# bluenote-1577/sylph

Measured on NVIDIA H100. Metric: bases/s sketched, higher is better.
Workload: dtype u64

## Files before the change

### sylph_b200/csrc/common.cuh

```cuda
#pragma once

#include <cuda_runtime.h>

#include <algorithm>
#include <stdint.h>
#include <stdio.h>

#include <string>
#include <unordered_map>
#include <utility>
#include <vector>

#include "../../include/sylph_b200.h"

namespace syl {

void set_error(const std::string &msg);

struct Status {
    int code;
    Status(int c = SYL_OK) : code(c) {}
    bool ok() const { return code == SYL_OK; }
};

#define SYL_CUDA(call)                                                                           \
    do {                                                                                         \
        cudaError_t _e = (call);                                                                 \
        if (_e != cudaSuccess) {                                                                 \
            ::syl::set_error(std::string(#call) + ": " + cudaGetErrorString(_e) + " (" +       \
                             __FILE__ + ":" + std::to_string(__LINE__) + ")");                   \
            return (_e == cudaErrorMemoryAllocation) ? SYL_ERR_OOM : SYL_ERR_CUDA;               \
        }                                                                                        \
    } while (0)

#define SYL_TRY(expr)                                                                            \
    do {                                                                                         \
        int _s = (expr);                                                                         \
        if (_s != SYL_OK) return _s;                                                             \
    } while (0)

}

struct syl_ctx {
    int device = 0;
    cudaStream_t stream = nullptr;
    bool own_stream = false;
    int num_sms = 132;
    uint64_t launches = 0;
    uint64_t *d_counters = nullptr;
    uint64_t *h_counters = nullptr;
    bool timing = false;
    struct TimedLaunch { int which; cudaEvent_t e0, e1; };
    std::vector<TimedLaunch> timed_pending;
    std::vector<cudaEvent_t> event_pool;
    double kernel_ms[SYL_KERNEL_COUNT] = {};
    uint64_t kernel_launches[SYL_KERNEL_COUNT] = {};
    uint64_t seed_bases = 0;
    uint64_t ingest_h2d_bytes = 0, ingest_chunks_packed = 0, ingest_chunks_ascii = 0;
    void *ingest = nullptr;
    cudaStream_t copy_stream = nullptr;
    cudaEvent_t ev_copied[2] = {nullptr, nullptr}, ev_used[2] = {nullptr, nullptr};
    uint8_t *stage_b[2] = {nullptr, nullptr};
    uint64_t *stage_o[2] = {nullptr, nullptr};
    uint64_t stage_cap_b[2] = {0, 0}, stage_cap_o[2] = {0, 0};
    std::vector<std::pair<void *, size_t>> free_blocks;
    std::unordered_map<void *, size_t> handle_blocks;
    size_t cached_bytes = 0;
};

namespace syl {
struct KernelTimer {
    syl_ctx *c;
    int which;
    cudaEvent_t e0 = nullptr, e1 = nullptr;
    KernelTimer(syl_ctx *ctx, int w) : c(ctx), which(w) {
        if (!c->timing) return;
        auto take = [&]() {
            cudaEvent_t e = nullptr;
            if (!c->event_pool.empty()) { e = c->event_pool.back(); c->event_pool.pop_back(); }
            else if (cudaEventCreate(&e) != cudaSuccess) e = nullptr;
            return e;
        };
        e0 = take(); e1 = take();
        if (e0 && e1) cudaEventRecord(e0, c->stream);
    }
    void stop() {
        if (!e0 || !e1) return;
        cudaEventRecord(e1, c->stream);
        c->timed_pending.push_back({which, e0, e1});
        e0 = e1 = nullptr;
    }
    ~KernelTimer() { stop(); }
};
extern thread_local syl_ctx *tl_ctx;
int hblock_alloc(syl_ctx *ctx, void **p, size_t bytes);
void hblock_free(syl_ctx *ctx, void *p);
}

struct syl_sample {
    int device = 0;
    syl_ctx *owner = nullptr;
    cudaStream_t stream = nullptr;
    uint64_t *hash = nullptr;
    uint32_t *count = nullptr;
    uint64_t n = 0;
    int k = 31;
    uint64_t c = 200;
    double mean_read_length = 0.;
    uint64_t num_dup_removed = 0;
    uint64_t sum_counts = 0;
    bool sum_counts_valid = false;
};

struct syl_genomes {
    int device = 0;
    syl_ctx *owner = nullptr;
    cudaStream_t stream = nullptr;
    uint64_t n = 0;
    uint64_t *kmers = nullptr, *kmer_off = nullptr;
    uint64_t *tracked = nullptr, *tracked_off = nullptr;
    uint64_t *gn_size = nullptr;
    uint64_t total_kmers = 0, total_tracked = 0;
    int has_tracked = 0;
    int k = 31;
    uint64_t c = 200;
};

namespace syl {

struct EventRec { uint64_t hash, recflag, p0, p1; };
static_assert(sizeof(EventRec) == 32, "EventRec is one 32-byte sector");
constexpr uint64_t NO_PAIR = 1ull;
constexpr uint64_t EV_PENDING = 1ull << 63;

constexpr uint32_t GRP_BPG = 32;

struct SeedJob {
    const uint8_t *d_bases = nullptr;
    const uint32_t *d_packed = nullptr;
    uint64_t n_bases = 0;
    const uint64_t *d_rec_off = nullptr;
    uint64_t off_bias = 0, n_rec = 0;
    int k = 31;
    uint64_t c = 200;
    int sem = SYL_SEM_AVX2, with_pos = 0;
    void *d_out = nullptr;
    uint64_t cap = 0;
    int emit_events = 0;
    uint64_t rec_base = 0;
    int no_dedup = 0;
    uint32_t *d_pend = nullptr;
    uint32_t *d_group_cnt = nullptr;
    uint64_t Mb = 0;
    uint32_t nbk = 0, ng = 0, slot = 0;
    unsigned long long *d_count = nullptr, *d_pend_count = nullptr;
    uint32_t slot_cap = 0;
    uint32_t *d_tile_cnt = nullptr, *d_slot_overflow = nullptr;
};
uint64_t seed_cta_tiles(uint64_t n_bases);
uint64_t seed_cta_tile_bases();
bool seed_cta_kernel_selected();
int seed_enqueue(syl_ctx *ctx, const SeedJob &job);
void ingest_destroy(syl_ctx *ctx);

template <typename T>
struct DevBuf {
    T *p = nullptr;
    size_t n = 0, cap_bytes = 0;
    cudaStream_t s = nullptr;
    syl_ctx *owner = nullptr;
    DevBuf() {}
    DevBuf(const DevBuf &) = delete;
    DevBuf &operator=(const DevBuf &) = delete;
    ~DevBuf() { release(); }
    int alloc(size_t count, cudaStream_t stream) {
        release();
        s = stream;
        n = count;
        size_t bytes = (std::max<size_t>(count, 1) * sizeof(T) + 255) & ~(size_t)255;
        syl_ctx *c = tl_ctx;
        owner = c;
        if (c) {
            size_t best = (size_t)-1, bi = 0;
            for (size_t i = 0; i < c->free_blocks.size(); i++) {
                const size_t sz = c->free_blocks[i].second;
                if (sz >= bytes && sz < best) { best = sz; bi = i; }
            }
            if (best != (size_t)-1 && best <= 2 * bytes + (1u << 20)) {
                p = reinterpret_cast<T *>(c->free_blocks[bi].first);
                cap_bytes = best;
                c->free_blocks[bi] = c->free_blocks.back();
                c->free_blocks.pop_back();
                return SYL_OK;
            }
        }
        cudaError_t e = cudaMalloc((void **)&p, bytes);
        if (e != cudaSuccess) {
            p = nullptr;
            set_error(std::string("cudaMalloc(") + std::to_string(bytes) + " B): " + cudaGetErrorString(e));
            return e == cudaErrorMemoryAllocation ? SYL_ERR_OOM : SYL_ERR_CUDA;
        }
        cap_bytes = bytes;
        if (c) c->cached_bytes += bytes;
        return SYL_OK;
    }
    void swap(DevBuf &o) {
        std::swap(p, o.p); std::swap(n, o.n); std::swap(cap_bytes, o.cap_bytes); std::swap(s, o.s); std::swap(owner, o.owner);
    }
    void release() {
        if (p) {
            if (owner) owner->free_blocks.emplace_back((void *)p, cap_bytes);
            else cudaFree(p);
        }
        p = nullptr;
        n = 0;
    }
};

__device__ __forceinline__ uint32_t even_fields(uint64_t x) {
    x &= 0xCCCCCCCCCCCCCCCCull;
    x = (x | (x << 2)) & 0xF0F0F0F0F0F0F0F0ull;
    x = (x | (x << 4)) & 0xFF00FF00FF00FF00ull;
    x = (x | (x << 8)) & 0xFFFF0000FFFF0000ull;
    x = (x | (x << 16)) & 0xFFFFFFFF00000000ull;
    return (uint32_t)(x >> 32);
}


__host__ __device__ __forceinline__ uint32_t byte_to_seq(uint32_t b) {
    switch (b) {
        case 1: case 'C': case 'c': return 1u;
        case 2: case 'G': case 'g': return 2u;
        case 3: case 'T': case 't': case 'U': case 'u': return 3u;
        default: return 0u;
    }
}

__host__ __device__ __forceinline__ uint64_t mm_hash64(uint64_t key) {
    key = ~(key * 0x200001ull);
    key ^= key >> 24;
    key *= 265ull;
    key ^= key >> 14;
    key *= 21ull;
    key ^= key >> 28;
    key *= 0x80000001ull;
    return key;
}

__host__ __device__ __forceinline__ uint64_t fmh_threshold(uint64_t c) {
    return 0xFFFFFFFFFFFFFFFFull / c;
}

__host__ __device__ __forceinline__ uint64_t valid_windows(uint64_t L, uint32_t k, int sem,
                                                           int with_pos) {
    if (L < k) return 0;
    if (sem == SYL_SEM_SCALAR) return L - k + 1;
    uint64_t min_len = with_pos ? 2ull * k : (uint64_t)k + 1;
    if (L < min_len) return 0;
    return 4ull * ((L - k + 1) / 4);
}

}
```

### sylph_b200/csrc/seed_kernel.cuh

```cuda
#pragma once
#include "common.cuh"

namespace syl {

constexpr int SEED_THREADS = 256;
#ifndef SEED_TILE_CFG
#define SEED_TILE_CFG 32768
#endif
#ifndef SEED_CANON_MODE
#define SEED_CANON_MODE 3
#endif
#ifndef SEED_MINB_CFG
#define SEED_MINB_CFG 4
#endif
constexpr int SEED_TILE = SEED_TILE_CFG;
constexpr int SEED_W_MAX = 32;
constexpr int SEED_W_MIN = 24;
constexpr int SEED_HALO = 48;
constexpr int SEED_STAGE = SEED_TILE >= 32768 ? 512 : 256;
constexpr int SEED_CAND = SEED_TILE >= 32768 ? 1024 : 512;
constexpr int SEED_RUNS_PER_THREAD = (SEED_TILE / SEED_W_MIN + 2 * SEED_THREADS - 1) / SEED_THREADS;
constexpr int SEED_MAXRUNS = SEED_THREADS * SEED_RUNS_PER_THREAD;
static_assert(SEED_MAXRUNS >= SEED_TILE / SEED_W_MIN + SEED_THREADS, "run table too small");
constexpr int SEED_ASC_BYTES = SEED_TILE + SEED_HALO;
constexpr int SEED_NCHUNK16 = SEED_ASC_BYTES / 16;
constexpr int SEED_FW_WORDS = SEED_NCHUNK16 + 1 + 8;
constexpr int SEED_CW_WORDS = SEED_NCHUNK16 + 8;

struct SeedSmem {
    alignas(128) uint8_t asc[SEED_ASC_BYTES + 16];
    alignas(16) uint32_t fw[SEED_FW_WORDS];
    alignas(16) uint32_t cw[SEED_CW_WORDS];
    alignas(16) uint8_t lut[4][256];
    alignas(8) unsigned long long mbar;
};
struct SeedMeta {
    long long rel[SEED_THREADS];
    int s0[SEED_THREADS];
    int cnt[SEED_THREADS];
    int len[SEED_THREADS];
    int rbase[SEED_THREADS + 1];
    int warp_tot[SEED_THREADS / 32];
    unsigned int stage_count;
    unsigned int cand_count;
    unsigned long long flush_base;
    alignas(16) EventRec stage[SEED_STAGE];
    uint32_t cand[SEED_CAND];
    uint16_t run_rec[SEED_MAXRUNS];
};
static_assert(sizeof(SeedMeta) <= SEED_ASC_BYTES, "meta must fit in the dead ASCII region");
static_assert(SEED_TILE <= 65536, "tile-relative window starts are kept as u16");
__device__ __forceinline__ uint16_t *seed_stage_pos(SeedMeta &M) {
    return reinterpret_cast<uint16_t *>(reinterpret_cast<syl_survivor *>(M.stage) + SEED_STAGE);
}

struct GroupOut {
    uint32_t *cnt;
    uint64_t Mb;
    uint32_t nbk, ng, slot;
    __device__ __forceinline__ uint64_t place(uint64_t h, unsigned long long *g_count, uint64_t cap) const {
        if (cnt) {
            uint32_t g = (uint32_t)__umul64hi(h, Mb);
            g = (g < nbk ? g : nbk - 1) / GRP_BPG;
            const uint32_t i = atomicAdd(&cnt[g], 1u);
            if (i < slot) return (uint64_t)g * slot + i;
        }
        const unsigned long long gi = atomicAdd(g_count, 1ull);
        return gi < cap ? (uint64_t)ng * slot + gi : ~0ull;
    }
};

struct ShiftMul { uint32_t m24, m14, m28, one, zero; };

struct SlotOut { uint32_t cap; uint32_t *tile_cnt; uint32_t *overflow; };

__device__ __forceinline__ void mul64c(uint32_t lo, uint32_t hi, uint32_t c, uint32_t &plo, uint32_t &phi) {
    uint64_t t;
    asm("mul.wide.u32 %0, %1, %2;" : "=l"(t) : "r"(lo), "r"(c));
    plo = (uint32_t)t;
    asm("mad.lo.u32 %0, %1, %2, %3;" : "=r"(phi) : "r"(hi), "r"(c), "r"((uint32_t)(t >> 32)));
}

template <int VAR, int SH>
__device__ __forceinline__ void xorshift(uint32_t &lo, uint32_t &hi, uint32_t mul, uint32_t extra_hi) {
    uint32_t sl, sh;
    if (VAR >= 1) sh = __umulhi(hi, mul); else sh = hi >> SH;
    if (VAR >= 2) sl = __umulhi(lo, mul) + hi * mul; else sl = __funnelshift_r(lo, hi, SH);
    lo ^= sl;
    hi = hi ^ sh ^ extra_hi;
}

template <int VAR>
__device__ __forceinline__ uint32_t hash_hi32(uint32_t lo, uint32_t hi, const ShiftMul sm) {
    uint32_t a, b;
    mul64c(lo, hi, 0x200001u, a, b);
    xorshift<VAR, 24>(a, b, sm.m24, 0xFFFFFF00u);
    mul64c(a, b, 265u, lo, hi);
    xorshift<VAR, 14>(lo, hi, sm.m14, 0u);
    mul64c(lo, hi, 21u, a, b);
    xorshift<VAR, 28>(a, b, sm.m28, 0u);
    return __umulhi(a, 0x80000001u) + b * 0x80000001u;
}

__device__ __forceinline__ uint32_t smem_u32(const void *p) {
    return (uint32_t)__cvta_generic_to_shared(p);
}

__device__ __forceinline__ uint64_t fw64(const SeedSmem &S, uint32_t q) {
    const uint32_t bitpos = 32u + 2u * q, w = bitpos >> 5, sh = bitpos & 31u;
    const uint32_t a = S.fw[w], b = S.fw[w + 1], c = S.fw[w + 2];
    return ((uint64_t)__funnelshift_l(b, a, sh) << 32) | __funnelshift_l(c, b, sh);
}

template <int K, int EMIT>
__device__ __forceinline__ void seed_resolve(const SeedSmem &S, SeedMeta &M, uint32_t pw, int j, uint64_t rc, uint64_t thr,
                                             void *__restrict__ out, uint64_t cap,
                                             unsigned long long *__restrict__ g_count, uint64_t rec_base, int no_dedup,
                                             uint32_t *__restrict__ pend, const GroupOut go) {
    constexpr uint32_t PAD = 64 - 2 * K;
    constexpr uint32_t HI_MASK = (1u << (32 - PAD)) - 1u;
    const uint32_t bitpos = 32u + 2u * pw - PAD;
    const uint32_t q0 = bitpos >> 5, sh = bitpos & 31u;
    const uint32_t w0 = S.fw[q0], w1 = S.fw[q0 + 1], w2 = S.fw[q0 + 2];
    const uint64_t f = ((uint64_t)(__funnelshift_l(w1, w0, sh) & HI_MASK) << 32) | __funnelshift_l(w2, w1, sh);
    const uint32_t cq = pw >> 4, csh = (pw & 15u) * 2u;
    const uint32_t c0 = S.cw[cq], c1 = S.cw[cq + 1], c2 = S.cw[cq + 2];
    const uint64_t rr = ((uint64_t)(__funnelshift_r(c1, c2, csh) & HI_MASK) << 32) | __funnelshift_r(c0, c1, csh);
    const uint64_t h = mm_hash64(f < rr ? f : rr);
    if (h >= thr) return;
    const unsigned int idx = atomicAdd(&M.stage_count, 1u);
    if (EMIT == 0) {
        syl_survivor sv;
        sv.hash = h;
        sv.rec = (uint32_t)(rc + (uint64_t)j);
        sv.pos = (uint32_t)((long long)pw - M.rel[j] + (K - 1));
        if (idx < (unsigned)SEED_STAGE) {
            reinterpret_cast<syl_survivor *>(M.stage)[idx] = sv;
            seed_stage_pos(M)[idx] = (uint16_t)pw;
        } else {
            const unsigned long long gi = atomicAdd(g_count, 1ull);
            if (gi < cap) reinterpret_cast<syl_survivor *>(out)[gi] = sv;
        }
    } else {
        EventRec ev;
        ev.hash = h;
        const int L = M.len[j];
        const bool has_pair = !no_dedup && L <= 400 && L >= 66;
        ev.recflag = ((rec_base + rc + (uint64_t)j) << 1) | (no_dedup == 2 ? EV_PENDING : (has_pair ? 0ull : NO_PAIR));
        ev.p0 = 0;
        ev.p1 = 0;
        if (has_pair) {
            const long long st = M.rel[j];
            const long long mid = st + (L >> 1);
            if (st >= 0 && mid + 32 <= (long long)SEED_NCHUNK16 * 16) {
                const uint64_t a = fw64(S, (uint32_t)st), b = fw64(S, (uint32_t)mid);
                const uint32_t kf = even_fields(a), kg = even_fields(a << 2);
                const uint32_t kr = even_fields(b), kt = even_fields(b << 2);
                ev.p0 = ((uint64_t)kf << 32) | kr;
                ev.p1 = ((uint64_t)kg << 32) | kt;
            } else {
                ev.recflag |= EV_PENDING;
            }
        }
        if (idx < (unsigned)SEED_STAGE) {
            M.stage[idx] = ev;
        } else {
            const uint64_t pos = go.place(ev.hash, g_count, cap);
            if (pos != ~0ull) {
                reinterpret_cast<EventRec *>(out)[pos] = ev;
                if (ev.recflag & EV_PENDING) pend[atomicAdd(g_count + 1, 1ull)] = (uint32_t)pos;
            }
        }
    }
}

template <int K, int VAR, int EMIT, int W>
__global__ void __launch_bounds__(SEED_THREADS, SEED_MINB_CFG)
k_seed(const uint8_t *__restrict__ bases, uint64_t n_bases, const uint64_t *__restrict__ rec_off, uint64_t off_bias,
       const uint32_t *__restrict__ tile_rec, uint64_t thr, int sem, int with_pos,
       void *__restrict__ out, uint64_t cap, unsigned long long *__restrict__ g_count,
       const ShiftMul smul, uint64_t rec_base, int no_dedup, uint32_t *__restrict__ pend, const GroupOut go, const SlotOut slot) {
    static_assert(W >= SEED_W_MIN && W <= SEED_W_MAX, "run length");
    extern __shared__ __align__(128) uint8_t smem_raw[];
    SeedSmem &S = *reinterpret_cast<SeedSmem *>(smem_raw);
    SeedMeta &M = *reinterpret_cast<SeedMeta *>(S.asc);

    constexpr uint32_t PAD = 64 - 2 * K;
    constexpr uint32_t HI_MASK = (1u << (32 - PAD)) - 1u;
    const int tid = threadIdx.x;
    const uint64_t T0 = (uint64_t)blockIdx.x * SEED_TILE;
    const uint64_t T1 = T0 + SEED_TILE;
    const uint32_t thr_hi = (uint32_t)(thr >> 32);

    const uint64_t remain = n_bases - T0;
    const uint32_t avail = remain < (uint64_t)SEED_ASC_BYTES ? (uint32_t)remain : (uint32_t)SEED_ASC_BYTES;
    const uint32_t nbulk = avail & ~15u;
    const uint32_t mbar = smem_u32(&S.mbar);
    if (tid == 0) {
        asm volatile("mbarrier.init.shared::cta.b64 [%0], 1;" ::"r"(mbar));
        asm volatile("fence.mbarrier_init.release.cluster;" ::: "memory");
    }
    __syncthreads();
    if (tid == 0 && nbulk) {
        asm volatile("mbarrier.arrive.expect_tx.shared::cta.b64 _, [%0], %1;" ::"r"(mbar), "r"(nbulk)
                     : "memory");
        asm volatile(
            "cp.async.bulk.shared::cluster.global.mbarrier::complete_tx::bytes [%0], [%1], %2, [%3];" ::"r"(
                smem_u32(S.asc)),
            "l"(bases + T0), "r"(nbulk), "r"(mbar)
            : "memory");
    }
    for (uint32_t i = nbulk + tid; i < (uint32_t)SEED_ASC_BYTES + 16; i += SEED_THREADS)
        S.asc[i] = (i < avail) ? bases[T0 + i] : (uint8_t)0;
    {
        const uint32_t code = byte_to_seq((uint32_t)tid);
        S.lut[0][tid] = (uint8_t)(code << 6);
        S.lut[1][tid] = (uint8_t)(code << 4);
        S.lut[2][tid] = (uint8_t)(code << 2);
        S.lut[3][tid] = (uint8_t)code;
    }
    if (tid < 8) {
        S.fw[SEED_NCHUNK16 + 1 + tid] = 0u;
        S.cw[SEED_NCHUNK16 + tid] = 0u;
    }
    if (tid == 0) S.fw[0] = 0u;
    if (nbulk) {
        uint32_t done = 0;
        while (!done) {
            asm volatile(
                "{\n\t.reg .pred p;\n\t"
                "mbarrier.try_wait.parity.shared::cta.b64 p, [%1], 0;\n\t"
                "selp.u32 %0, 1, 0, p;\n\t}"
                : "=r"(done)
                : "r"(mbar)
                : "memory");
        }
    }
    __syncthreads();

    for (int ch = tid; ch < SEED_NCHUNK16; ch += SEED_THREADS) {
        const uint4 v = *reinterpret_cast<const uint4 *>(S.asc + 16 * ch);
        const uint32_t w[4] = {v.x, v.y, v.z, v.w};
        uint32_t g[4];
#pragma unroll
        for (int q = 0; q < 4; q++) {
            const uint32_t b0 = __byte_perm(w[q], 0u, 0x4440), b1 = __byte_perm(w[q], 0u, 0x4441);
            const uint32_t b2 = __byte_perm(w[q], 0u, 0x4442), b3 = __byte_perm(w[q], 0u, 0x4443);
            g[q] = ((uint32_t)S.lut[0][b0] | (uint32_t)S.lut[1][b1] | (uint32_t)S.lut[2][b2]) | (uint32_t)S.lut[3][b3];
        }
        const uint32_t lo16 = __byte_perm(g[3], g[2], 0x0040), hi16 = __byte_perm(g[1], g[0], 0x0040);
        const uint32_t f = __byte_perm(lo16, hi16, 0x5410);
        uint32_t x = __brev(f);
        x = ((x >> 1) & 0x55555555u) | ((x & 0x55555555u) << 1);
        S.fw[1 + ch] = f;
        S.cw[ch] = ~x;
    }
    __syncthreads();

    if (tid == 0) M.stage_count = 0u;

    const uint32_t r_lo = tile_rec[blockIdx.x];
    const uint32_t r_hi = tile_rec[blockIdx.x + 1];
    const int lane = tid & 31, wid = tid >> 5;

    for (uint64_t rc = r_lo; rc <= (uint64_t)r_hi; rc += SEED_THREADS) {
        int runs = 0;
        const uint64_t r = rc + tid;
        if (r <= (uint64_t)r_hi) {
            const uint64_t a = rec_off[r] - off_bias, b = rec_off[r + 1] - off_bias;
            const uint64_t L = b - a;
            const uint64_t nv = valid_windows(L, (uint32_t)K, sem, with_pos);
            const uint64_t lo = a > T0 ? a : T0;
            uint64_t hi = a + nv;
            if (hi > T1) hi = T1;
            const int cnt = hi > lo ? (int)(hi - lo) : 0;
            M.rel[tid] = (long long)a - (long long)T0;
            M.s0[tid] = (int)(lo - T0);
            M.cnt[tid] = cnt;
            M.len[tid] = L > 0x7FFFFFFFull ? 0x7FFFFFFF : (int)L;
            runs = (cnt + W - 1) / W;
        }
        int incl = runs;
#pragma unroll
        for (int d = 1; d < 32; d <<= 1) {
            int t = __shfl_up_sync(0xffffffffu, incl, d);
            if (lane >= d) incl += t;
        }
        if (lane == 31) M.warp_tot[wid] = incl;
        __syncthreads();
        int wbase = 0;
#pragma unroll
        for (int w = 0; w < SEED_THREADS / 32; w++) wbase += (w < wid) ? M.warp_tot[w] : 0;
        M.rbase[tid] = wbase + incl - runs;
        if (tid == SEED_THREADS - 1) M.rbase[SEED_THREADS] = wbase + incl;
        __syncthreads();
        const int total = M.rbase[SEED_THREADS];

        {
            const int base5 = tid * SEED_RUNS_PER_THREAD;
#pragma unroll
            for (int e = 0; e < SEED_RUNS_PER_THREAD; e++) M.run_rec[base5 + e] = 0;
            __syncthreads();
            if (runs > 0) M.run_rec[M.rbase[tid]] = (uint16_t)(tid + 1);
            __syncthreads();
            int v[SEED_RUNS_PER_THREAD], m = 0;
#pragma unroll
            for (int e = 0; e < SEED_RUNS_PER_THREAD; e++) { m = max(m, (int)M.run_rec[base5 + e]); v[e] = m; }
            int inc = m;
#pragma unroll
            for (int d = 1; d < 32; d <<= 1) inc = max(inc, __shfl_up_sync(0xffffffffu, inc, d));
            int excl = __shfl_up_sync(0xffffffffu, inc, 1);
            if (lane == 0) excl = 0;
            if (lane == 31) M.warp_tot[wid] = inc;
            __syncthreads();
            int wmax = 0;
#pragma unroll
            for (int w = 0; w < SEED_THREADS / 32; w++) wmax = max(wmax, (w < wid) ? M.warp_tot[w] : 0);
            const int pre = max(excl, wmax);
#pragma unroll
            for (int e = 0; e < SEED_RUNS_PER_THREAD; e++) M.run_rec[base5 + e] = (uint16_t)max(v[e], pre);
            if (tid == 0) M.cand_count = 0u;
            __syncthreads();
        }

        for (int q = tid; q < total; q += SEED_THREADS) {
            const int j = (int)M.run_rec[q] - 1;
            const int ridx = q - M.rbase[j];
            const int p = M.s0[j] + ridx * W;
            const int n = min(W, M.cnt[j] - ridx * W);

            uint32_t F[4], G[4];
            {
                const uint32_t bitpos = 32u + 2u * (uint32_t)p - PAD;
                const uint32_t q0 = bitpos >> 5, sh = bitpos & 31u;
                uint32_t w0 = S.fw[q0], w1 = S.fw[q0 + 1], w2 = S.fw[q0 + 2], w3 = S.fw[q0 + 3],
                         w4 = S.fw[q0 + 4];
                F[0] = __funnelshift_l(w1, w0, sh);
                F[1] = __funnelshift_l(w2, w1, sh);
                F[2] = __funnelshift_l(w3, w2, sh);
                F[3] = __funnelshift_l(w4, w3, sh);
                const uint32_t cq = (uint32_t)p >> 4, csh = ((uint32_t)p & 15u) * 2u;
                uint32_t c0 = S.cw[cq], c1 = S.cw[cq + 1], c2 = S.cw[cq + 2], c3 = S.cw[cq + 3],
                         c4 = S.cw[cq + 4];
                G[0] = __funnelshift_r(c0, c1, csh);
                G[1] = __funnelshift_r(c1, c2, csh);
                G[2] = __funnelshift_r(c2, c3, csh);
                G[3] = __funnelshift_r(c3, c4, csh);
            }
            uint32_t cand = 0u;
#pragma unroll
            for (int i = 0; i < W; i++) {
                const int jb = (2 * i) >> 5;
                const uint32_t sft = (uint32_t)((2 * i) & 31);
                const uint32_t f_hi = __funnelshift_l(F[jb + 1], F[jb], sft) & HI_MASK;
                const uint32_t f_lo = __funnelshift_l(F[jb + 2], F[jb + 1], sft);
                const uint32_t r_lo = __funnelshift_r(G[jb], G[jb + 1], sft);
                const uint32_t r_hi = __funnelshift_r(G[jb + 1], G[jb + 2], sft) & HI_MASK;
                uint32_t c_lo, c_hi;
#if SEED_CANON_MODE == 0
                const uint64_t f = ((uint64_t)f_hi << 32) | f_lo, rr = ((uint64_t)r_hi << 32) | r_lo;
                const uint64_t canon = f < rr ? f : rr;
                c_lo = (uint32_t)canon; c_hi = (uint32_t)(canon >> 32);
#elif SEED_CANON_MODE == 1
                asm("{\n\t.reg .pred p;\n\t.reg .f64 a, b;\n\tmov.b64 a, {%2, %3};\n\tmov.b64 b, {%4, %5};\n\t"
                    "setp.lt.f64 p, a, b;\n\tselp.b32 %0, %2, %4, p;\n\tselp.b32 %1, %3, %5, p;\n\t}"
                    : "=r"(c_lo), "=r"(c_hi) : "r"(f_lo), "r"(f_hi), "r"(r_lo), "r"(r_hi));
#else
                c_lo = r_lo; c_hi = r_hi;
                asm("{\n\t.reg .pred p;\n\t.reg .f64 a, b;\n\tmov.b64 a, {%2, %3};\n\tmov.b64 b, {%4, %5};\n\t"
                    "setp.lt.f64 p, a, b;\n\t@p mad.lo.u32 %0, %2, %6, %7;\n\t@p mad.lo.u32 %1, %3, %6, %7;\n\t}"
                    : "+r"(c_lo), "+r"(c_hi) : "r"(f_lo), "r"(f_hi), "r"(r_lo), "r"(r_hi), "r"(smul.one), "r"(smul.zero));
#endif
                const uint32_t hh = hash_hi32<VAR>(c_lo, c_hi, smul);
#if SEED_CANON_MODE >= 3
                asm("{\n\t.reg .pred p;\n\tsetp.le.u32 p, %1, %2;\n\t@p mad.lo.u32 %0, %3, %4, %0;\n\t}"
                    : "+r"(cand) : "r"(hh), "r"(thr_hi), "r"(smul.one), "r"(1u << i));
#else
                asm("{\n\t.reg .pred p;\n\tsetp.le.u32 p, %1, %2;\n\t@p or.b32 %0, %0, %3;\n\t}"
                    : "+r"(cand) : "r"(hh), "r"(thr_hi), "r"(1u << i));
#endif
            }
            if (n < W) cand &= (1u << n) - 1u;
            while (cand) {
                const int i = __ffs(cand) - 1;
                cand &= cand - 1u;
                const unsigned int ci = atomicAdd(&M.cand_count, 1u);
                if (ci < (unsigned)SEED_CAND) {
                    M.cand[ci] = ((uint32_t)(p + i) << 8) | (uint32_t)j;
                } else {
                    seed_resolve<K, EMIT>(S, M, (uint32_t)(p + i), j, rc, thr, out, cap, g_count, rec_base, no_dedup, pend, go);
                }
            }
        }
        __syncthreads();
        {
            const unsigned int nc = min(M.cand_count, (unsigned)SEED_CAND);
            for (unsigned int ci = tid; ci < nc; ci += SEED_THREADS) {
                const uint32_t e = M.cand[ci];
                seed_resolve<K, EMIT>(S, M, e >> 8, (int)(e & 255u), rc, thr, out, cap, g_count, rec_base, no_dedup, pend, go);
            }
        }
        __syncthreads();
    }

    __syncthreads();
    if (EMIT == 0 && slot.cap) {
        const unsigned int total = M.stage_count;
        const unsigned int lim = min((unsigned)SEED_STAGE, slot.cap);
        const unsigned int nst = min(total, lim);
        if (tid == 0) {
            slot.tile_cnt[blockIdx.x] = nst;
            if (total > lim) atomicExch(slot.overflow, 1u);
        }
        constexpr int NW = SEED_TILE / 32, PER = NW / SEED_THREADS;
        static_assert(NW % SEED_THREADS == 0 && NW <= SEED_CW_WORDS, "bitmap layout");
        uint32_t *bits = S.fw, *pre = S.cw;
        const uint16_t *sp = seed_stage_pos(M);
        for (int i = tid; i < NW; i += SEED_THREADS) bits[i] = 0u;
        __syncthreads();
        for (unsigned int i = tid; i < nst; i += SEED_THREADS) atomicOr(&bits[sp[i] >> 5], 1u << (sp[i] & 31u));
        __syncthreads();
        {
            uint32_t cnt[PER], tot = 0;
#pragma unroll
            for (int e = 0; e < PER; e++) { cnt[e] = __popc(bits[PER * tid + e]); tot += cnt[e]; }
            uint32_t inc = tot;
#pragma unroll
            for (int d = 1; d < 32; d <<= 1) { const uint32_t v = __shfl_up_sync(0xffffffffu, inc, d); if ((tid & 31) >= d) inc += v; }
            if ((tid & 31) == 31) M.warp_tot[tid >> 5] = (int)inc;
            __syncthreads();
            uint32_t base = inc - tot;
            for (int w = 0; w < (tid >> 5); w++) base += (uint32_t)M.warp_tot[w];
#pragma unroll
            for (int e = 0; e < PER; e++) { pre[PER * tid + e] = base; base += cnt[e]; }
        }
        __syncthreads();
        syl_survivor *dst = reinterpret_cast<syl_survivor *>(out) + (uint64_t)blockIdx.x * slot.cap;
        for (unsigned int i = tid; i < nst; i += SEED_THREADS) {
            const uint32_t p = sp[i], w = p >> 5;
            dst[pre[w] + __popc(bits[w] & ((1u << (p & 31u)) - 1u))] = reinterpret_cast<const syl_survivor *>(M.stage)[i];
        }
        return;
    }
    const unsigned int staged = min(M.stage_count, (unsigned)SEED_STAGE);
    if (EMIT == 1 && go.cnt) {
        for (unsigned int i = tid; i < staged; i += SEED_THREADS) {
            const EventRec ev = M.stage[i];
            const uint64_t pos = go.place(ev.hash, g_count, cap);
            if (pos == ~0ull) continue;
            reinterpret_cast<EventRec *>(out)[pos] = ev;
            if (ev.recflag & EV_PENDING) pend[atomicAdd(g_count + 1, 1ull)] = (uint32_t)pos;
        }
        return;
    }
    if (tid == 0 && staged) M.flush_base = atomicAdd(g_count, (unsigned long long)staged);
    __syncthreads();
    if (staged) {
        const unsigned long long base = M.flush_base;
        for (unsigned int i = tid; i < staged; i += SEED_THREADS) {
            if (base + i >= cap) continue;
            if (EMIT == 0) reinterpret_cast<syl_survivor *>(out)[base + i] = reinterpret_cast<const syl_survivor *>(M.stage)[i];
            else {
                const EventRec ev = M.stage[i];
                reinterpret_cast<EventRec *>(out)[base + i] = ev;
                if (ev.recflag & EV_PENDING) pend[atomicAdd(g_count + 1, 1ull)] = (uint32_t)(base + i);
            }
        }
    }
}


using seed_kern_t = void (*)(const uint8_t *, uint64_t, const uint64_t *, uint64_t, const uint32_t *, uint64_t, int, int,
                             void *, uint64_t, unsigned long long *, const ShiftMul, uint64_t, int, uint32_t *, const GroupOut, const SlotOut);

#define SEED_DEFINE_KERNELS(NAME, K, EMIT)                            \
    seed_kern_t NAME(int W) {                                         \
        switch (W) {                                                  \
            case 24: return k_seed<K, 0, EMIT, 24>;                   \
            case 30: return k_seed<K, 0, EMIT, 30>;                   \
            default: return k_seed<K, 0, EMIT, 32>;                   \
        }                                                             \
    }

seed_kern_t seed_kernels_k31_sv(int W);
seed_kern_t seed_kernels_k31_ev(int W);
seed_kern_t seed_kernels_k21_sv(int W);
seed_kern_t seed_kernels_k21_ev(int W);

}
```

Measured before the change: 455.1 billion.

## Add direct run-record scatter path and move LUT to static shared memory

Adds a fast path to the run-offset scan. When no thread has more than a small number of runs, each thread writes its run records directly, which skips the zero-fill, max-scan and extra barriers. The block total is now computed from the warp totals, dropping one barrier and the extra rbase slot. The byte-to-code LUT now lives in static shared memory and is filled from a packed constant table, and the LUT lookups are combined with adds instead of ORs. The hash xorshift variant template is split per stage, which looks like a generalisation of the variant parameter.

After: 472.3 billion, median of 6. +3.8%, better.

```diff
diff --git a/sylph_b200/csrc/common.cuh b/sylph_b200/csrc/common.cuh
--- a/sylph_b200/csrc/common.cuh
+++ b/sylph_b200/csrc/common.cuh
@@ -227,7 +227,7 @@
 }
 
 
-__host__ __device__ __forceinline__ uint32_t byte_to_seq(uint32_t b) {
+__host__ __device__ __forceinline__ constexpr uint32_t byte_to_seq(uint32_t b) {
     switch (b) {
         case 1: case 'C': case 'c': return 1u;
         case 2: case 'G': case 'g': return 2u;
diff --git a/sylph_b200/csrc/seed_kernel.cuh b/sylph_b200/csrc/seed_kernel.cuh
--- a/sylph_b200/csrc/seed_kernel.cuh
+++ b/sylph_b200/csrc/seed_kernel.cuh
@@ -31,16 +31,23 @@
     alignas(128) uint8_t asc[SEED_ASC_BYTES + 16];
     alignas(16) uint32_t fw[SEED_FW_WORDS];
     alignas(16) uint32_t cw[SEED_CW_WORDS];
-    alignas(16) uint8_t lut[4][256];
     alignas(8) unsigned long long mbar;
 };
+struct ByteToSeq2 { uint32_t w[16]; };
+constexpr ByteToSeq2 byte_to_seq2() {
+    ByteToSeq2 t{};
+    for (uint32_t b = 0; b < 256; b++) t.w[b >> 4] |= byte_to_seq(b) << (2 * (b & 15));
+    return t;
+}
+static __constant__ ByteToSeq2 c_byte_to_seq2 = byte_to_seq2();
+constexpr int SEED_DIRECT_RUNS = 8;
 struct SeedMeta {
     long long rel[SEED_THREADS];
     int s0[SEED_THREADS];
     int cnt[SEED_THREADS];
     int len[SEED_THREADS];
-    int rbase[SEED_THREADS + 1];
-    int warp_tot[SEED_THREADS / 32];
+    int rbase[SEED_THREADS];
+    alignas(16) int warp_tot[SEED_THREADS / 32];
     unsigned int stage_count;
     unsigned int cand_count;
     unsigned long long flush_base;
@@ -94,11 +101,11 @@
 __device__ __forceinline__ uint32_t hash_hi32(uint32_t lo, uint32_t hi, const ShiftMul sm) {
     uint32_t a, b;
     mul64c(lo, hi, 0x200001u, a, b);
-    xorshift<VAR, 24>(a, b, sm.m24, 0xFFFFFF00u);
+    xorshift<VAR & 3, 24>(a, b, sm.m24, 0xFFFFFF00u);
     mul64c(a, b, 265u, lo, hi);
-    xorshift<VAR, 14>(lo, hi, sm.m14, 0u);
+    xorshift<(VAR >> 2) & 3, 14>(lo, hi, sm.m14, 0u);
     mul64c(lo, hi, 21u, a, b);
-    xorshift<VAR, 28>(a, b, sm.m28, 0u);
+    xorshift<(VAR >> 4) & 3, 28>(a, b, sm.m28, 0u);
     return __umulhi(a, 0x80000001u) + b * 0x80000001u;
 }
 
@@ -184,6 +191,7 @@
     extern __shared__ __align__(128) uint8_t smem_raw[];
     SeedSmem &S = *reinterpret_cast<SeedSmem *>(smem_raw);
     SeedMeta &M = *reinterpret_cast<SeedMeta *>(S.asc);
+    __shared__ __align__(16) uint8_t lut[4][256];
 
     constexpr uint32_t PAD = 64 - 2 * K;
     constexpr uint32_t HI_MASK = (1u << (32 - PAD)) - 1u;
@@ -213,11 +221,11 @@
     for (uint32_t i = nbulk + tid; i < (uint32_t)SEED_ASC_BYTES + 16; i += SEED_THREADS)
         S.asc[i] = (i < avail) ? bases[T0 + i] : (uint8_t)0;
     {
-        const uint32_t code = byte_to_seq((uint32_t)tid);
-        S.lut[0][tid] = (uint8_t)(code << 6);
-        S.lut[1][tid] = (uint8_t)(code << 4);
-        S.lut[2][tid] = (uint8_t)(code << 2);
-        S.lut[3][tid] = (uint8_t)code;
+        const uint32_t code = (c_byte_to_seq2.w[tid >> 4] >> (2 * (tid & 15))) & 3u;
+        lut[0][tid] = (uint8_t)(code << 6);
+        lut[1][tid] = (uint8_t)(code << 4);
+        lut[2][tid] = (uint8_t)(code << 2);
+        lut[3][tid] = (uint8_t)code;
     }
     if (tid < 8) {
         S.fw[SEED_NCHUNK16 + 1 + tid] = 0u;
@@ -246,7 +254,7 @@
         for (int q = 0; q < 4; q++) {
             const uint32_t b0 = __byte_perm(w[q], 0u, 0x4440), b1 = __byte_perm(w[q], 0u, 0x4441);
             const uint32_t b2 = __byte_perm(w[q], 0u, 0x4442), b3 = __byte_perm(w[q], 0u, 0x4443);
-            g[q] = ((uint32_t)S.lut[0][b0] | (uint32_t)S.lut[1][b1] | (uint32_t)S.lut[2][b2]) | (uint32_t)S.lut[3][b3];
+            g[q] = ((uint32_t)lut[0][b0] + (uint32_t)lut[1][b1]) + ((uint32_t)lut[2][b2] + (uint32_t)lut[3][b3]);
         }
         const uint32_t lo16 = __byte_perm(g[3], g[2], 0x0040), hi16 = __byte_perm(g[1], g[0], 0x0040);
         const uint32_t f = __byte_perm(lo16, hi16, 0x5410);
@@ -287,21 +295,28 @@
             if (lane >= d) incl += t;
         }
         if (lane == 31) M.warp_tot[wid] = incl;
-        __syncthreads();
-        int wbase = 0;
-#pragma unroll
-        for (int w = 0; w < SEED_THREADS / 32; w++) wbase += (w < wid) ? M.warp_tot[w] : 0;
-        M.rbase[tid] = wbase + incl - runs;
-        if (tid == SEED_THREADS - 1) M.rbase[SEED_THREADS] = wbase + incl;
-        __syncthreads();
-        const int total = M.rbase[SEED_THREADS];
-
-        {
+        const bool direct = !__syncthreads_or(runs > SEED_DIRECT_RUNS);
+        int wbase = 0, total = 0;
+#pragma unroll
+        for (int w = 0; w < SEED_THREADS / 32; w++) {
+            const int t = M.warp_tot[w];
+            wbase += (w < wid) ? t : 0;
+            total += t;
+        }
+        const int rb = wbase + incl - runs;
+        M.rbase[tid] = rb;
+        if (tid == 0) M.cand_count = 0u;
+
+        if (direct) {
+#pragma unroll 1
+            for (int e = 0; e < runs; e++) M.run_rec[rb + e] = (uint16_t)(tid + 1);
+            __syncthreads();
+        } else {
             const int base5 = tid * SEED_RUNS_PER_THREAD;
 #pragma unroll
             for (int e = 0; e < SEED_RUNS_PER_THREAD; e++) M.run_rec[base5 + e] = 0;
             __syncthreads();
-            if (runs > 0) M.run_rec[M.rbase[tid]] = (uint16_t)(tid + 1);
+            if (runs > 0) M.run_rec[rb] = (uint16_t)(tid + 1);
             __syncthreads();
             int v[SEED_RUNS_PER_THREAD], m = 0;
 #pragma unroll
@@ -319,7 +334,6 @@
             const int pre = max(excl, wmax);
 #pragma unroll
             for (int e = 0; e < SEED_RUNS_PER_THREAD; e++) M.run_rec[base5 + e] = (uint16_t)max(v[e], pre);
-            if (tid == 0) M.cand_count = 0u;
             __syncthreads();
         }
 
@@ -469,7 +483,6 @@
     }
 }
 
-
 using seed_kern_t = void (*)(const uint8_t *, uint64_t, const uint64_t *, uint64_t, const uint32_t *, uint64_t, int, int,
                              void *, uint64_t, unsigned long long *, const ShiftMul, uint64_t, int, uint32_t *, const GroupOut, const SlotOut);
 
```
